# lucidrains/progen

Measured on NVIDIA H100. Metric: tokens_per_sec, higher is better.
Workload: dtype bf16

## Files before the change

### progen_b200/csrc/attn_wgmma.cu

```cuda
#include <cuda.h>
#include "common.cuh"
#include "tc_ptx.cuh"
#include "../../include/progen_b200.h"

namespace {

using namespace tc;

constexpr int DH = 64;
constexpr int TILE = 64;
constexpr int TILE_BYTES = TILE * DH * 2;
constexpr float LOG2E = 1.4426950408889634f;
constexpr float LN2 = 0.6931471805599453f;
constexpr int SMEM_BYTES = 1024  + 2 * TILE_BYTES + 2 * 2 * TILE_BYTES + 64;

struct Dims {
  int n, w, h;
  const float* rot_sin;
  const float* rot_cos;
};

__device__ __forceinline__ float quad_max(float v) {
  v = fmaxf(v, __shfl_xor_sync(0xffffffffu, v, 1));
  return fmaxf(v, __shfl_xor_sync(0xffffffffu, v, 2));
}
__device__ __forceinline__ float quad_sum(float v) {
  v += __shfl_xor_sync(0xffffffffu, v, 1);
  return v + __shfl_xor_sync(0xffffffffu, v, 2);
}
__device__ __forceinline__ uint32_t unrotate_pack(const Dims& dm, int pos, int jj, float d0, float d1) {
  if (dm.rot_sin) {
    const float s = __ldg(dm.rot_sin + pos * (DH / 2) + jj), c = __ldg(dm.rot_cos + pos * (DH / 2) + jj);
    const float a = d0 * c + d1 * s, b = d1 * c - d0 * s;
    d0 = a; d1 = b;
  }
  return pack_bf16x2(d0, d1);
}
template <int R> __device__ __forceinline__ void zero(float (&a)[R]) {
#pragma unroll
  for (int i = 0; i < R; ++i) a[i] = 0.f;
}
__device__ __forceinline__ void acc_to_a(uint32_t (&a)[4][4], const float (&s)[32]) {
#pragma unroll
  for (int kk = 0; kk < 4; ++kk)
#pragma unroll
    for (int i = 0; i < 4; ++i) a[kk][i] = pack_bf16x2(s[8 * kk + 2 * i], s[8 * kk + 2 * i + 1]);
}
__device__ __forceinline__ void issue_a_xt(float (&acc)[32], uint32_t a, uint32_t x) {
#pragma unroll
  for (int kk = 0; kk < 4; ++kk) wgmma_m64n64k16_ss<0>(acc, make_smem_desc<false>(a + 32 * kk), make_smem_desc<false>(x + 32 * kk));
}
__device__ __forceinline__ void issue_p_x(float (&acc)[32], const uint32_t (&p)[4][4], uint32_t x) {
#pragma unroll
  for (int kk = 0; kk < 4; ++kk) wgmma_m64n64k16_rs<1>(acc, p[kk], make_smem_desc<true>(x + 2048 * kk));
}
template <int R> __device__ __forceinline__ void mma_begin(float (&acc)[R]) {
  fence_regs(acc);
  wgmma_fence();
}
template <int R> __device__ __forceinline__ void mma_end(float (&acc)[R]) {
  wgmma_commit();
  wgmma_wait<0>();
  fence_regs(acc);
}

struct Smem {
  uint32_t fixed0, fixed1, ring, bars;
  __device__ Smem(uint8_t* raw) {
    fixed0 = (smem_u32(raw) + 1023u) & ~1023u;
    fixed1 = fixed0 + TILE_BYTES;
    ring = fixed1 + TILE_BYTES;
    bars = ring + 4 * TILE_BYTES;
  }
  __device__ uint32_t a(int st) const { return ring + st * 2 * TILE_BYTES; }
  __device__ uint32_t b(int st) const { return a(st) + TILE_BYTES; }
  __device__ uint32_t fixed_bar() const { return bars; }
  __device__ uint32_t full(int st) const { return bars + 8 + 8 * st; }
};

__device__ __forceinline__ void init_bars(const Smem& sm) {
  if (threadIdx.x == 0) {
    mbar_init(sm.fixed_bar(), 1);
    mbar_init(sm.full(0), 1);
    mbar_init(sm.full(1), 1);
    fence_barrier_init();
  }
  __syncthreads();
}

__global__ void __launch_bounds__(128) attn_fwd_wgmma_kernel(const __grid_constant__ CUtensorMap tm_qkv, bf16* __restrict__ out,
                                                             float* __restrict__ lse, const Dims dm) {
  extern __shared__ uint8_t smem_raw[];
  const Smem sm(smem_raw);
  const int tid = threadIdx.x, lane = tid & 31, warp = tid >> 5;
  const int g = lane >> 2, t4 = lane & 3;
  const int b = blockIdx.z, hh = blockIdx.y;
  const int q0 = blockIdx.x * TILE, win = q0 / dm.w, i0 = q0 % dm.w;
  const int I = dm.h * DH;
  const int row0 = b * dm.n;
  const int nprev = win > 0 ? dm.w / TILE : 0;
  const int ntiles = nprev + (i0 + TILE) / TILE;
  auto key_pos = [&](int kt) { return kt < nprev ? (win - 1) * dm.w + kt * TILE : win * dm.w + (kt - nprev) * TILE; };
  auto issue = [&](int kt, int st) {
    mbar_expect_tx(sm.full(st), 2 * TILE_BYTES);
    tma_load_2d(sm.a(st), &tm_qkv, sm.full(st), I + hh * DH, row0 + key_pos(kt));
    tma_load_2d(sm.b(st), &tm_qkv, sm.full(st), 2 * I + hh * DH, row0 + key_pos(kt));
  };
  init_bars(sm);
  if (tid == 0) {
    prefetch_tensormap(&tm_qkv);
    mbar_expect_tx(sm.fixed_bar(), TILE_BYTES);
    tma_load_2d(sm.fixed0, &tm_qkv, sm.fixed_bar(), hh * DH, row0 + q0);
    for (int kt = 0; kt < 2 && kt < ntiles; ++kt) issue(kt, kt);
  }

  const float sc = 0.125f  * LOG2E;
  float m_run[2], l_run[2];
  m_run[0] = m_run[1] = (win == 0) ? 0.f : -INFINITY;
  l_run[0] = l_run[1] = (win == 0) ? (float)dm.w : 0.f;
  float o[32];
  zero(o);
  const int qi_lo = i0 + warp * 16;
  mbar_wait(sm.fixed_bar(), 0);

  for (int kt = 0; kt < ntiles; ++kt) {
    const int st = kt & 1;
    mbar_wait(sm.full(st), (kt >> 1) & 1);
    float s[32];
    zero(s);
    mma_begin(s);
    issue_a_xt(s, sm.fixed0, sm.a(st));
    mma_end(s);
    const int c0 = (kt - nprev) * TILE;
    const bool need_mask = kt >= nprev && c0 + TILE - 1 > qi_lo;
    float tmax[2] = {-INFINITY, -INFINITY};
#pragma unroll
    for (int i = 0; i < 32; ++i) {
      float v = s[i] * sc;
      if (need_mask) {
        const int kj = c0 + 8 * (i >> 2) + 2 * t4 + (i & 1);
        const int qi = qi_lo + g + (((i >> 1) & 1) << 3);
        if (kj > qi) v = -INFINITY;
      }
      s[i] = v;
      tmax[(i >> 1) & 1] = fmaxf(tmax[(i >> 1) & 1], v);
    }
    float corr[2], rsum[2] = {0.f, 0.f};
#pragma unroll
    for (int r = 0; r < 2; ++r) {
      const float mn = fmaxf(m_run[r], quad_max(tmax[r]));
      corr[r] = exp2f(m_run[r] - mn);
      m_run[r] = mn;
    }
#pragma unroll
    for (int i = 0; i < 32; ++i) {
      const float p = exp2f(s[i] - m_run[(i >> 1) & 1]);
      s[i] = p;
      rsum[(i >> 1) & 1] += p;
    }
#pragma unroll
    for (int r = 0; r < 2; ++r) l_run[r] = l_run[r] * corr[r] + quad_sum(rsum[r]);
#pragma unroll
    for (int i = 0; i < 32; ++i) o[i] *= corr[(i >> 1) & 1];
    uint32_t pa[4][4];
    acc_to_a(pa, s);
    mma_begin(o);
    issue_p_x(o, pa, sm.b(st));
    mma_end(o);
    __syncthreads();
    if (tid == 0 && kt + 2 < ntiles) {
      fence_proxy_async();
      issue(kt + 2, st);
    }
  }
#pragma unroll
  for (int r = 0; r < 2; ++r) {
    const long long t = (long long)row0 + q0 + warp * 16 + g + 8 * r;
    const float inv = 1.f / l_run[r];
    bf16* op = out + t * I + hh * DH + 2 * t4;
#pragma unroll
    for (int j = 0; j < 8; ++j)
      *reinterpret_cast<uint32_t*>(op + 8 * j) = pack_bf16x2(o[4 * j + 2 * r] * inv, o[4 * j + 2 * r + 1] * inv);
    if (t4 == 0) lse[t * dm.h + hh] = m_run[r] * LN2 + logf(l_run[r]);
  }
}

__global__ void __launch_bounds__(128) attn_bwd_dq_wgmma_kernel(const __grid_constant__ CUtensorMap tm_qkv,
                                                                const __grid_constant__ CUtensorMap tm_do,
                                                                const bf16* __restrict__ out, const bf16* __restrict__ dout,
                                                                const float* __restrict__ lse, float* __restrict__ delta,
                                                                bf16* __restrict__ dqkv, const Dims dm) {
  extern __shared__ uint8_t smem_raw[];
  const Smem sm(smem_raw);
  const int tid = threadIdx.x, lane = tid & 31, warp = tid >> 5;
  const int g = lane >> 2, t4 = lane & 3;
  const int b = blockIdx.z, hh = blockIdx.y;
  const int q0 = blockIdx.x * TILE, win = q0 / dm.w, i0 = q0 % dm.w;
  const int I = dm.h * DH;
  const long long ld = 3LL * I;
  const int row0 = b * dm.n;
  const int nprev = win > 0 ? dm.w / TILE : 0;
  const int ntiles = nprev + (i0 + TILE) / TILE;
  auto key_pos = [&](int kt) { return kt < nprev ? (win - 1) * dm.w + kt * TILE : win * dm.w + (kt - nprev) * TILE; };
  auto issue = [&](int kt, int st) {
    mbar_expect_tx(sm.full(st), 2 * TILE_BYTES);
    tma_load_2d(sm.a(st), &tm_qkv, sm.full(st), I + hh * DH, row0 + key_pos(kt));
    tma_load_2d(sm.b(st), &tm_qkv, sm.full(st), 2 * I + hh * DH, row0 + key_pos(kt));
  };
  init_bars(sm);
  if (tid == 0) {
    prefetch_tensormap(&tm_qkv);
    prefetch_tensormap(&tm_do);
    mbar_expect_tx(sm.fixed_bar(), 2 * TILE_BYTES);
    tma_load_2d(sm.fixed0, &tm_qkv, sm.fixed_bar(), hh * DH, row0 + q0);
    tma_load_2d(sm.fixed1, &tm_do, sm.fixed_bar(), hh * DH, row0 + q0);
    for (int kt = 0; kt < 2 && kt < ntiles; ++kt) issue(kt, kt);
  }

  const float scale = 0.125f ;
  const float sc = scale * LOG2E;
  float L2[2], Dl[2];
#pragma unroll
  for (int r = 0; r < 2; ++r) {
    const long long t = (long long)row0 + q0 + warp * 16 + g + 8 * r;
    L2[r] = lse[t * dm.h + hh] * LOG2E;
    float acc = 0.f;
#pragma unroll
    for (int j = 0; j < 8; ++j) {
      const uint32_t ov = *reinterpret_cast<const uint32_t*>(out + t * I + hh * DH + 8 * j + 2 * t4);
      const uint32_t dv = *reinterpret_cast<const uint32_t*>(dout + t * I + hh * DH + 8 * j + 2 * t4);
      const float2 fo = __bfloat1622float2(*reinterpret_cast<const __nv_bfloat162*>(&ov));
      const float2 fd = __bfloat1622float2(*reinterpret_cast<const __nv_bfloat162*>(&dv));
      acc += fo.x * fd.x + fo.y * fd.y;
    }
    Dl[r] = quad_sum(acc);
    if (t4 == 0) delta[t * dm.h + hh] = Dl[r];
  }
  float dq[32];
  zero(dq);
  const int qi_lo = i0 + warp * 16;
  mbar_wait(sm.fixed_bar(), 0);

  for (int kt = 0; kt < ntiles; ++kt) {
    const int st = kt & 1;
    mbar_wait(sm.full(st), (kt >> 1) & 1);
    float s[32], dp[32];
    zero(s);
    zero(dp);
    fence_regs(dp);
    mma_begin(s);
    issue_a_xt(s, sm.fixed0, sm.a(st));
    issue_a_xt(dp, sm.fixed1, sm.b(st));
    mma_end(s);
    fence_regs(dp);
    const int c0 = (kt - nprev) * TILE;
    const bool need_mask = kt >= nprev && c0 + TILE - 1 > qi_lo;
#pragma unroll
    for (int i = 0; i < 32; ++i) {
      const int r = (i >> 1) & 1;
      float p = exp2f(s[i] * sc - L2[r]);
      if (need_mask) {
        const int kj = c0 + 8 * (i >> 2) + 2 * t4 + (i & 1);
        const int qi = qi_lo + g + (r << 3);
        if (kj > qi) p = 0.f;
      }
      s[i] = p * (dp[i] - Dl[r]) * scale;
    }
    uint32_t dsa[4][4];
    acc_to_a(dsa, s);
    mma_begin(dq);
    issue_p_x(dq, dsa, sm.a(st));
    mma_end(dq);
    __syncthreads();
    if (tid == 0 && kt + 2 < ntiles) {
      fence_proxy_async();
      issue(kt + 2, st);
    }
  }
#pragma unroll
  for (int r = 0; r < 2; ++r) {
    const int pos = q0 + warp * 16 + g + 8 * r;
    bf16* op = dqkv + ((long long)row0 + pos) * ld + hh * DH + 2 * t4;
#pragma unroll
    for (int j = 0; j < 8; ++j)
      *reinterpret_cast<uint32_t*>(op + 8 * j) = unrotate_pack(dm, pos, 4 * j + t4, dq[4 * j + 2 * r], dq[4 * j + 2 * r + 1]);
  }
}

__global__ void __launch_bounds__(128) attn_bwd_dkv_wgmma_kernel(const __grid_constant__ CUtensorMap tm_qkv,
                                                                 const __grid_constant__ CUtensorMap tm_do,
                                                                 const float* __restrict__ lse, const float* __restrict__ delta,
                                                                 bf16* __restrict__ dqkv, const Dims dm) {
  extern __shared__ uint8_t smem_raw[];
  const Smem sm(smem_raw);
  const int tid = threadIdx.x, lane = tid & 31, warp = tid >> 5;
  const int g = lane >> 2, t4 = lane & 3;
  const int b = blockIdx.z, hh = blockIdx.y;
  const int k0 = blockIdx.x * TILE, win = k0 / dm.w, j0 = k0 % dm.w;
  const int I = dm.h * DH;
  const long long ld = 3LL * I;
  const int row0 = b * dm.n;
  const int nwin = (dm.n + dm.w - 1) / dm.w;
  const int own_end = min((win + 1) * dm.w, dm.n);
  const int nown = (own_end - k0) / TILE;
  const int nnext = (win + 1 < nwin) ? (min((win + 2) * dm.w, dm.n) - own_end) / TILE : 0;
  const int ntiles = nown + nnext;
  auto q_pos = [&](int qt) { return qt < nown ? win * dm.w + j0 + qt * TILE : (win + 1) * dm.w + (qt - nown) * TILE; };
  auto issue = [&](int qt, int st) {
    mbar_expect_tx(sm.full(st), 2 * TILE_BYTES);
    tma_load_2d(sm.a(st), &tm_qkv, sm.full(st), hh * DH, row0 + q_pos(qt));
    tma_load_2d(sm.b(st), &tm_do, sm.full(st), hh * DH, row0 + q_pos(qt));
  };
  init_bars(sm);
  if (tid == 0) {
    prefetch_tensormap(&tm_qkv);
    prefetch_tensormap(&tm_do);
    mbar_expect_tx(sm.fixed_bar(), 2 * TILE_BYTES);
    tma_load_2d(sm.fixed0, &tm_qkv, sm.fixed_bar(), I + hh * DH, row0 + k0);
    tma_load_2d(sm.fixed1, &tm_qkv, sm.fixed_bar(), 2 * I + hh * DH, row0 + k0);
    for (int qt = 0; qt < 2 && qt < ntiles; ++qt) issue(qt, qt);
  }

  const float scale = 0.125f ;
  const float sc = scale * LOG2E;
  float dk[32], dv[32];
  zero(dk);
  zero(dv);
  const int kj_lo = j0 + warp * 16;
  mbar_wait(sm.fixed_bar(), 0);

  for (int qt = 0; qt < ntiles; ++qt) {
    const int st = qt & 1;
    const int qp = q_pos(qt);
    float Lq[16], Dq[16];
#pragma unroll
    for (int j = 0; j < 8; ++j)
#pragma unroll
      for (int c = 0; c < 2; ++c) {
        const long long t = (long long)row0 + qp + 8 * j + 2 * t4 + c;
        Lq[2 * j + c] = __ldg(lse + t * dm.h + hh) * LOG2E;
        Dq[2 * j + c] = __ldg(delta + t * dm.h + hh);
      }
    mbar_wait(sm.full(st), (qt >> 1) & 1);
    float s[32], dp[32];
    zero(s);
    zero(dp);
    fence_regs(dp);
    mma_begin(s);
    issue_a_xt(s, sm.fixed0, sm.a(st));
    issue_a_xt(dp, sm.fixed1, sm.b(st));
    mma_end(s);
    fence_regs(dp);
    const bool own = qt < nown;
    const int c0 = j0 + qt * TILE;
    const bool need_mask = own && c0 < kj_lo + 15;
#pragma unroll
    for (int i = 0; i < 32; ++i) {
      const int col = 8 * (i >> 2) + 2 * t4 + (i & 1);
      const int ci = 2 * (i >> 2) + (i & 1);
      float p = exp2f(s[i] * sc - Lq[ci]);
      if (need_mask) {
        const int qi = c0 + col;
        const int kj = kj_lo + g + (((i >> 1) & 1) << 3);
        if (kj > qi) p = 0.f;
      }
      dp[i] = p * (dp[i] - Dq[ci]) * scale;
      s[i] = p;
    }
    uint32_t pa[4][4], dsa[4][4];
    acc_to_a(pa, s);
    acc_to_a(dsa, dp);
    fence_regs(dk);
    mma_begin(dv);
    issue_p_x(dv, pa, sm.b(st));
    issue_p_x(dk, dsa, sm.a(st));
    mma_end(dv);
    fence_regs(dk);
    __syncthreads();
    if (tid == 0 && qt + 2 < ntiles) {
      fence_proxy_async();
      issue(qt + 2, st);
    }
  }
#pragma unroll
  for (int r = 0; r < 2; ++r) {
    const int pos = k0 + warp * 16 + g + 8 * r;
    bf16* pk = dqkv + ((long long)row0 + pos) * ld + I + hh * DH + 2 * t4;
    bf16* pv = pk + I;
#pragma unroll
    for (int j = 0; j < 8; ++j) {
      *reinterpret_cast<uint32_t*>(pk + 8 * j) = unrotate_pack(dm, pos, 4 * j + t4, dk[4 * j + 2 * r], dk[4 * j + 2 * r + 1]);
      *reinterpret_cast<uint32_t*>(pv + 8 * j) = unrotate_pack(dm, pos, 4 * j + t4, dv[4 * j + 2 * r], dv[4 * j + 2 * r + 1]);
    }
  }
}

template <typename K> int prepare(K kern) {
  static bool done = false;
  if (!done) {
    PG_CUDA(cudaFuncSetAttribute(kern, cudaFuncAttributeMaxDynamicSharedMemorySize, SMEM_BYTES));
    done = true;
  }
  return PROGEN_OK;
}

int check_dims(const void* qkv, int B, int seq_len, int window, int heads, int dim_head, bool full_windows) {
  PG_CHECK_ARG(qkv != nullptr && B > 0 && heads > 0 && dim_head == DH && window % TILE == 0 && seq_len > 0 &&
               seq_len % (full_windows ? window : TILE) == 0);
  PG_CHECK_ARG((long long)B * seq_len < (1ll << 31));
  return PROGEN_OK;
}

int bwd_tc(const void* qkv, const void* out, const void* dout, const float* lse, void* dqkv, float* delta,
           const float* rot_sin, const float* rot_cos, int B, int seq_len, int window, int heads, cudaStream_t s) {
  int rc;
  const int I = heads * DH;
  const uint64_t T = (uint64_t)B * seq_len;
  CUtensorMap tq, tdo;
  if ((rc = pg_tensor_map_2d_bf16(qkv, 3ull * I, T, 3ull * I, DH, TILE, &tq))) return rc;
  if ((rc = pg_tensor_map_2d_bf16(dout, (uint64_t)I, T, (uint64_t)I, DH, TILE, &tdo))) return rc;
  if ((rc = prepare(attn_bwd_dq_wgmma_kernel))) return rc;
  if ((rc = prepare(attn_bwd_dkv_wgmma_kernel))) return rc;
  const Dims dm{seq_len, window, heads, rot_sin, rot_cos};
  const dim3 grid(seq_len / TILE, heads, B);
  attn_bwd_dq_wgmma_kernel<<<grid, 128, SMEM_BYTES, s>>>(tq, tdo, (const bf16*)out, (const bf16*)dout, lse, delta, (bf16*)dqkv, dm);
  PG_LAUNCH_CHECK();
  attn_bwd_dkv_wgmma_kernel<<<grid, 128, SMEM_BYTES, s>>>(tq, tdo, lse, delta, (bf16*)dqkv, dm);
  PG_LAUNCH_CHECK();
  return PROGEN_OK;
}

}

extern "C" {

int progen_local_attn_fwd_tc(const void* qkv, void* out, float* lse, int B, int seq_len, int window, int heads, int dim_head,
                             void* stream) {
  int rc = check_dims(qkv, B, seq_len, window, heads, dim_head, false);
  if (rc) return rc;
  const int I = heads * DH;
  const uint64_t T = (uint64_t)B * seq_len;
  CUtensorMap tm;
  if ((rc = pg_tensor_map_2d_bf16(qkv, 3ull * I, T, 3ull * I, DH, TILE, &tm))) return rc;
  if ((rc = prepare(attn_fwd_wgmma_kernel))) return rc;
  const Dims dm{seq_len, window, heads, nullptr, nullptr};
  attn_fwd_wgmma_kernel<<<dim3(seq_len / TILE, heads, B), 128, SMEM_BYTES, (cudaStream_t)stream>>>(tm, (bf16*)out, lse, dm);
  PG_LAUNCH_CHECK();
  return PROGEN_OK;
}

int progen_local_attn_bwd_tc(const void* qkv, const void* out, const void* dout, const float* lse, void* dqkv, float* delta,
                             const float* rot_sin, const float* rot_cos, int B, int seq_len, int window, int heads, int dim_head,
                             void* stream) {
  const int rc = check_dims(qkv, B, seq_len, window, heads, dim_head, true);
  return rc ? rc : bwd_tc(qkv, out, dout, lse, dqkv, delta, rot_sin, rot_cos, B, seq_len, window, heads, (cudaStream_t)stream);
}

int progen_local_attn_bwd_cut_tc(const void* qkv, const void* out, const void* dout, const float* lse, void* dqkv,
                                 float* delta, const float* rot_sin, const float* rot_cos, int B, int seq_len, int window,
                                 int heads, int dim_head, void* stream) {
  const int rc = check_dims(qkv, B, seq_len, window, heads, dim_head, false);
  return rc ? rc : bwd_tc(qkv, out, dout, lse, dqkv, delta, rot_sin, rot_cos, B, seq_len, window, heads, (cudaStream_t)stream);
}

}
```

### progen_b200/csrc/gemm_tc.cu

```cuda
#include <cuda.h>
#include <algorithm>
#include <mutex>
#include <unordered_map>
#include "gemm.h"
#include "tc_ptx.cuh"

namespace {

using namespace tc;

constexpr int BM = 128;
constexpr int BN = 128;
constexpr int BK = 64;
constexpr int WG_K = 16;
constexpr int THREADS = 384;
constexpr int A_BYTES = BM * BK * 2;
constexpr int B_BYTES = BN * BK * 2;
constexpr int STAGE_BYTES = A_BYTES + B_BYTES;
constexpr int STAGES = 4;
constexpr int EPI_ROWS = 64;
constexpr int EPI_ITEMS = EPI_ROWS * (BN / 8) / 128;
constexpr int CS_LD = BN + 4;
constexpr int CS_BYTES = EPI_ROWS * CS_LD * 4;
constexpr int SMEM_TOTAL = 1024  + STAGES * STAGE_BYTES + 2 * CS_BYTES + 2 * STAGES * 8;
// ... 265 lines not shown

EncodeTiledFn get_encode_fn() {
  static EncodeTiledFn fn = nullptr;
  static std::once_flag once;
  std::call_once(once, [] {
    void* p = nullptr;
    cudaDriverEntryPointQueryResult q;
    if (cudaGetDriverEntryPoint("cuTensorMapEncodeTiled", &p, cudaEnableDefault, &q) == cudaSuccess &&
        q == cudaDriverEntryPointSuccess)
      fn = reinterpret_cast<EncodeTiledFn>(p);
  });
  return fn;
}

struct MapKey {
  const void* ptr; uint64_t inner, outer, stride; uint32_t box_inner, box_outer, elem_bytes, swizzle;
  bool operator==(const MapKey& o) const {
    return ptr == o.ptr && inner == o.inner && outer == o.outer && stride == o.stride && box_inner == o.box_inner &&
           box_outer == o.box_outer && elem_bytes == o.elem_bytes && swizzle == o.swizzle;
  }
};
struct MapKeyHash {
  size_t operator()(const MapKey& k) const {
    size_t h = std::hash<const void*>()(k.ptr);
    auto mix = [&](uint64_t v) { h ^= std::hash<uint64_t>()(v) + 0x9e3779b97f4a7c15ULL + (h << 6) + (h >> 2); };
    mix(k.inner); mix(k.outer); mix(k.stride); mix(k.box_inner); mix(k.box_outer); mix(k.elem_bytes * 256 + k.swizzle);
    return h;
  }
};

int get_tensor_map(const void* ptr, uint64_t inner, uint64_t outer, uint64_t row_stride_elems, uint32_t box_inner,
                   uint32_t box_outer, CUtensorMap* out, uint32_t elem_bytes = 2, uint32_t swizzle = 128) {
  static std::unordered_map<MapKey, CUtensorMap, MapKeyHash> cache;
  static std::mutex mu;
  MapKey key{ptr, inner, outer, row_stride_elems, box_inner, box_outer, elem_bytes, swizzle};
  std::lock_guard<std::mutex> lock(mu);
  auto it = cache.find(key);
  if (it != cache.end()) { *out = it->second; return PROGEN_OK; }
  EncodeTiledFn fn = get_encode_fn();
  if (!fn) { progen_set_error("cuTensorMapEncodeTiled driver entry point not found"); return PROGEN_ERR_DEVICE; }
  cuuint64_t dims[2] = {inner, outer};
  cuuint64_t strides[1] = {row_stride_elems * elem_bytes};
  const CUtensorMapSwizzle sw = swizzle == 128 ? CU_TENSOR_MAP_SWIZZLE_128B : swizzle == 64 ? CU_TENSOR_MAP_SWIZZLE_64B
                              : swizzle == 32 ? CU_TENSOR_MAP_SWIZZLE_32B : CU_TENSOR_MAP_SWIZZLE_NONE;
  cuuint32_t box[2] = {box_inner, box_outer};
  cuuint32_t estr[2] = {1, 1};
  CUtensorMap m;
  CUresult r = fn(&m, elem_bytes == 4 ? CU_TENSOR_MAP_DATA_TYPE_FLOAT32 : CU_TENSOR_MAP_DATA_TYPE_BFLOAT16, 2,
                  const_cast<void*>(ptr), dims, strides, box, estr, CU_TENSOR_MAP_INTERLEAVE_NONE, sw, CU_TENSOR_MAP_L2_PROMOTION_L2_256B,
                  CU_TENSOR_MAP_FLOAT_OOB_FILL_NONE);
  if (r != CUDA_SUCCESS) {
    progen_set_error("cuTensorMapEncodeTiled failed (CUresult %d) ptr=%p inner=%llu outer=%llu stride=%llu box=%ux%u", (int)r,
                     ptr, (unsigned long long)inner, (unsigned long long)outer, (unsigned long long)row_stride_elems,
                     box_inner, box_outer);
    return PROGEN_ERR_CUDA;
  }
  if (cache.size() > 4096) cache.clear();
  cache.emplace(key, m);
  *out = m;
  return PROGEN_OK;
}


template <bool A_MN, bool B_MN, int KIND, typename TO, bool TAIL>
int launch_inst(const CUtensorMap& ta, const CUtensorMap& tb, const CUtensorMap& ta2, const CUtensorMap& tb2,
                const GemmDev& gd, int tiles, cudaStream_t stream) {
  auto kern = gemm_tc_kernel<A_MN, B_MN, KIND, TO, TAIL>;
  static bool attr_set = false;
  if (!attr_set) {
    PG_CUDA(cudaFuncSetAttribute(kern, cudaFuncAttributeMaxDynamicSharedMemorySize, SMEM_TOTAL));
    attr_set = true;
  }
  kern<<<std::min(tiles, pg_num_sms()), THREADS, SMEM_TOTAL, stream>>>(ta, tb, ta2, tb2, gd, tiles);
  PG_LAUNCH_CHECK();
  return PROGEN_OK;
}

}

int pg_tensor_map_2d_bf16(const void* ptr, uint64_t inner, uint64_t outer, uint64_t row_stride_elems, uint32_t box_inner,
                          uint32_t box_outer, CUtensorMap* out) {
  return get_tensor_map(ptr, inner, outer, row_stride_elems, box_inner, box_outer, out);
}

int gemm_tc_launch(const GemmArgs& a, cudaStream_t stream) {
  PG_CHECK_ARG(a.in_dtype == PG_BF16);
  PG_CHECK_ARG(a.M > 0 && a.N > 0 && a.K > 0 && a.batch >= 1 && a.split_k >= 1);
  PG_CHECK_ARG(a.N % 8 == 0);
  PG_CHECK_ARG(a.K % BK == 0);
  PG_CHECK_ARG(a.lda % 8 == 0 && a.ldb % 8 == 0);
  PG_CHECK_ARG((reinterpret_cast<uintptr_t>(a.A) & 15) == 0 && (reinterpret_cast<uintptr_t>(a.B) & 15) == 0);
  PG_CHECK_ARG(!(a.split_k > 1 && a.causal));
  if (a.epi_kind == EPI_ROTARY) PG_CHECK_ARG(a.epi.seq_len % 32 == 0);
  PG_CHECK_ARG((reinterpret_cast<uintptr_t>(a.epi.colsum) & 15) == 0);
  PG_CHECK_ARG(!(a.split_k > 1 || a.batch_reduce) || (a.epi_kind == EPI_ACCUM && a.epi.atomic));
  PG_CHECK_TAIL(a);
  const bool tail = a.K2 > 0;
  if (tail) {
    PG_CHECK_ARG(a.K2 % 8 == 0 && a.lda2 % 8 == 0 && a.ldb2 % 8 == 0);
    PG_CHECK_ARG(a.a2_mn_major == a.a_mn_major && a.b2_mn_major == a.b_mn_major);
    PG_CHECK_ARG((reinterpret_cast<uintptr_t>(a.A2) & 15) == 0 && (reinterpret_cast<uintptr_t>(a.B2) & 15) == 0);
  }

  const uint64_t a_rows = (a.batch > 1 && a.a_batch_rows > 0) ? (uint64_t)a.a_batch_rows * a.batch
                                                              : (uint64_t)(a.a_mn_major ? a.K : a.M);
  const uint64_t b_rows = (a.batch > 1 && a.b_batch_rows > 0) ? (uint64_t)a.b_batch_rows * a.batch
                                                              : (uint64_t)(a.b_mn_major ? a.K : a.N);
  CUtensorMap ta, tb;
  int rc;
  if (!a.a_mn_major) rc = get_tensor_map(a.A, a.K, a_rows, a.lda, BK, BM, &ta);
  else               rc = get_tensor_map(a.A, a.M, a_rows, a.lda, 64, BK, &ta);
  if (rc) return rc;
  if (!a.b_mn_major) rc = get_tensor_map(a.B, a.K, b_rows, a.ldb, BK, BN, &tb);
  else               rc = get_tensor_map(a.B, a.N, b_rows, a.ldb, 64, BK, &tb);
  if (rc) return rc;
  CUtensorMap ta2 = ta, tb2 = tb;
  if (tail) {
    if (!a.a_mn_major) rc = get_tensor_map(a.A2, a.K2, a.M, a.lda2, BK, BM, &ta2);
    else               rc = get_tensor_map(a.A2, a.M, a.K2, a.lda2, 64, BK, &ta2);
    if (rc) return rc;
    if (!a.b_mn_major) rc = get_tensor_map(a.B2, a.K2, a.N, a.ldb2, BK, BN, &tb2);
    else               rc = get_tensor_map(a.B2, a.N, a.K2, a.ldb2, 64, BK, &tb2);
    if (rc) return rc;
  }

  GemmDev gd;
  gd.M = a.M; gd.N = a.N; gd.K = a.K;
  gd.batch = a.batch; gd.batch_reduce = a.batch_reduce;
  gd.a_batch_rows = (int)a.a_batch_rows; gd.b_batch_rows = (int)a.b_batch_rows; gd.d_batch_rows = a.d_batch_rows;
  gd.causal = a.causal; gd.split_k = a.split_k;
  gd.epi = a.epi;
  gd.K2 = a.K2;
  const long long tiles = (long long)a.batch * a.split_k * ((a.M + BM - 1) / BM) * ((a.N + BN - 1) / BN);
  PG_CHECK_ARG(tiles < (1ll << 31));

  const int am = a.a_mn_major ? 1 : 0, bm = a.b_mn_major ? 1 : 0;
  const bool obf = a.out_dtype == PG_BF16;
#define TC_CASE(AM, BMJ, KIND, TO)                                                                       \
  return tail ? launch_inst<AM, BMJ, KIND, TO, true>(ta, tb, ta2, tb2, gd, (int)tiles, stream)            \
              : launch_inst<AM, BMJ, KIND, TO, false>(ta, tb, ta2, tb2, gd, (int)tiles, stream)
  switch (a.epi_kind) {
    case EPI_STORE:
      if (!am && bm) { if (obf) TC_CASE(false, true, EPI_STORE, bf16); else TC_CASE(false, true, EPI_STORE, float); }
      if (!am && !bm) { if (obf) TC_CASE(false, false, EPI_STORE, bf16); else TC_CASE(false, false, EPI_STORE, float); }
      if (am && bm) { if (obf) TC_CASE(true, true, EPI_STORE, bf16); else TC_CASE(true, true, EPI_STORE, float); }
      break;
    case EPI_ROTARY:
      if (!am && bm && obf) TC_CASE(false, true, EPI_ROTARY, bf16);
      break;
    case EPI_RESIDUAL:
      if (!am && bm) TC_CASE(false, true, EPI_RESIDUAL, float);
      break;
    case EPI_GLU:
      if (!am && bm && obf) TC_CASE(false, true, EPI_GLU, bf16);
      break;
    case EPI_GELU:
      if (!am && bm && obf) TC_CASE(false, true, EPI_GELU, bf16);
      break;
    case EPI_GLU_BWD:
      if (!am && !bm && obf) TC_CASE(false, false, EPI_GLU_BWD, bf16);
      break;
    case EPI_GELU_BWD:
      if (!am && !bm && obf) TC_CASE(false, false, EPI_GELU_BWD, bf16);
      break;
    case EPI_ACCUM:
      if (am && bm) return launch_inst<true, true, EPI_ACCUM, float, false>(ta, tb, ta2, tb2, gd, (int)tiles, stream);
// ... 9 lines not shown
```

### progen_b200/csrc/tc_ptx.cuh

```cuda
#pragma once
#include <cuda.h>
#include "common.cuh"

namespace tc {

__device__ __forceinline__ uint32_t smem_u32(const void* p) { return (uint32_t)__cvta_generic_to_shared(p); }

__device__ __forceinline__ void mbar_init(uint32_t bar, uint32_t count) {
  asm volatile("mbarrier.init.shared::cta.b64 [%0], %1;" ::"r"(bar), "r"(count) : "memory");
}
__device__ __forceinline__ void mbar_expect_tx(uint32_t bar, uint32_t bytes) {
  asm volatile("mbarrier.arrive.expect_tx.shared::cta.b64 _, [%0], %1;" ::"r"(bar), "r"(bytes) : "memory");
}
__device__ __forceinline__ void mbar_arrive(uint32_t bar) {
  asm volatile("mbarrier.arrive.shared::cta.b64 _, [%0];" ::"r"(bar) : "memory");
}
__device__ __forceinline__ void mbar_wait(uint32_t bar, uint32_t parity) {
  uint32_t ok = 0, spins = 0;
  do {
    asm volatile(
        "{\n\t.reg .pred p;\n\t"
        "mbarrier.try_wait.parity.shared::cta.b64 p, [%1], %2;\n\t"
        "selp.u32 %0, 1, 0, p;\n\t}"
        : "=r"(ok) : "r"(bar), "r"(parity) : "memory");
    if (!ok && ++spins > (1u << 26)) __trap();
  } while (!ok);
}
__device__ __forceinline__ void fence_barrier_init() { asm volatile("fence.mbarrier_init.release.cluster;" ::: "memory"); }
__device__ __forceinline__ void fence_proxy_async() { asm volatile("fence.proxy.async.shared::cta;" ::: "memory"); }

__device__ __forceinline__ void tma_load_2d(uint32_t dst, const CUtensorMap* map, uint32_t bar, int c0, int c1) {
  asm volatile(
      "cp.async.bulk.tensor.2d.shared::cluster.global.mbarrier::complete_tx::bytes [%0], [%1, {%3, %4}], [%2];"
      ::"r"(dst), "l"(map), "r"(bar), "r"(c0), "r"(c1) : "memory");
}
__device__ __forceinline__ void prefetch_tensormap(const CUtensorMap* map) {
  asm volatile("prefetch.tensormap [%0];" ::"l"(map) : "memory");
}

template <bool MN_MAJOR>
__device__ __forceinline__ uint64_t make_smem_desc(uint32_t smem_addr, uint32_t lbo_bytes = 8192) {
  uint64_t d = 0;
  d |= (uint64_t)((smem_addr & 0x3FFFF) >> 4);
  d |= (uint64_t)(MN_MAJOR ? (lbo_bytes >> 4) : 1) << 16;
  d |= (uint64_t)(1024 >> 4) << 32;
  d |= (uint64_t)1 << 62;
  return d;
}

__device__ __forceinline__ void wgmma_fence() { asm volatile("wgmma.fence.sync.aligned;" ::: "memory"); }
__device__ __forceinline__ void wgmma_commit() { asm volatile("wgmma.commit_group.sync.aligned;" ::: "memory"); }
template <int N> __device__ __forceinline__ void wgmma_wait() { asm volatile("wgmma.wait_group.sync.aligned %0;" ::"n"(N) : "memory"); }
template <int R> __device__ __forceinline__ void fence_regs(float (&d)[R]) {
#pragma unroll
  for (int i = 0; i < R; ++i) asm volatile("" : "+f"(d[i])::"memory");
}

template <int TA, int TB>
__device__ __forceinline__ void wgmma_m64n128k16_bf16(float (&d)[64], uint64_t adesc, uint64_t bdesc) {
  asm volatile(
      "{\n\t"
      "wgmma.mma_async.sync.aligned.m64n128k16.f32.bf16.bf16 "
      "{%0, %1, %2, %3, %4, %5, %6, %7, %8, %9, %10, %11, %12, %13, %14, %15, %16, %17, %18, %19, %20, %21, %22, %23, "
      "%24, %25, %26, %27, %28, %29, %30, %31, %32, %33, %34, %35, %36, %37, %38, %39, %40, %41, %42, %43, %44, %45, %46, "
      "%47, %48, %49, %50, %51, %52, %53, %54, %55, %56, %57, %58, %59, %60, %61, %62, %63}, "
      "%64, %65, 1, 1, 1, %66, %67;\n\t}"
      : "+f"(d[0]), "+f"(d[1]), "+f"(d[2]), "+f"(d[3]), "+f"(d[4]), "+f"(d[5]), "+f"(d[6]), "+f"(d[7]), "+f"(d[8]),
        "+f"(d[9]), "+f"(d[10]), "+f"(d[11]), "+f"(d[12]), "+f"(d[13]), "+f"(d[14]), "+f"(d[15]), "+f"(d[16]),
        "+f"(d[17]), "+f"(d[18]), "+f"(d[19]), "+f"(d[20]), "+f"(d[21]), "+f"(d[22]), "+f"(d[23]), "+f"(d[24]),
        "+f"(d[25]), "+f"(d[26]), "+f"(d[27]), "+f"(d[28]), "+f"(d[29]), "+f"(d[30]), "+f"(d[31]), "+f"(d[32]),
        "+f"(d[33]), "+f"(d[34]), "+f"(d[35]), "+f"(d[36]), "+f"(d[37]), "+f"(d[38]), "+f"(d[39]), "+f"(d[40]),
        "+f"(d[41]), "+f"(d[42]), "+f"(d[43]), "+f"(d[44]), "+f"(d[45]), "+f"(d[46]), "+f"(d[47]), "+f"(d[48]),
        "+f"(d[49]), "+f"(d[50]), "+f"(d[51]), "+f"(d[52]), "+f"(d[53]), "+f"(d[54]), "+f"(d[55]), "+f"(d[56]),
        "+f"(d[57]), "+f"(d[58]), "+f"(d[59]), "+f"(d[60]), "+f"(d[61]), "+f"(d[62]), "+f"(d[63])
      : "l"(adesc), "l"(bdesc), "n"(TA), "n"(TB));
}

template <int TB>
__device__ __forceinline__ void wgmma_m64n64k16_ss(float (&d)[32], uint64_t adesc, uint64_t bdesc) {
  asm volatile(
      "{\n\t"
      "wgmma.mma_async.sync.aligned.m64n64k16.f32.bf16.bf16 "
      "{%0, %1, %2, %3, %4, %5, %6, %7, %8, %9, %10, %11, %12, %13, %14, %15, %16, %17, %18, %19, %20, %21, %22, %23, %24, %25, %26, %27, %28, %29, %30, %31}, "
      "%32, %33, 1, 1, 1, 0, %34;\n\t}"
      : "+f"(d[0]), "+f"(d[1]), "+f"(d[2]), "+f"(d[3]), "+f"(d[4]), "+f"(d[5]), "+f"(d[6]), "+f"(d[7]), "+f"(d[8]), "+f"(d[9]), "+f"(d[10]), "+f"(d[11]), "+f"(d[12]), "+f"(d[13]), "+f"(d[14]), "+f"(d[15]), "+f"(d[16]), "+f"(d[17]), "+f"(d[18]), "+f"(d[19]), "+f"(d[20]), "+f"(d[21]), "+f"(d[22]), "+f"(d[23]), "+f"(d[24]), "+f"(d[25]), "+f"(d[26]), "+f"(d[27]), "+f"(d[28]), "+f"(d[29]), "+f"(d[30]), "+f"(d[31])
      : "l"(adesc), "l"(bdesc), "n"(TB));
}
template <int TB>
__device__ __forceinline__ void wgmma_m64n64k16_rs(float (&d)[32], const uint32_t (&a)[4], uint64_t bdesc) {
  asm volatile(
      "{\n\t"
      "wgmma.mma_async.sync.aligned.m64n64k16.f32.bf16.bf16 "
      "{%0, %1, %2, %3, %4, %5, %6, %7, %8, %9, %10, %11, %12, %13, %14, %15, %16, %17, %18, %19, %20, %21, %22, %23, %24, %25, %26, %27, %28, %29, %30, %31}, "
      "{%32, %33, %34, %35}, %36, 1, 1, 1, %37;\n\t}"
      : "+f"(d[0]), "+f"(d[1]), "+f"(d[2]), "+f"(d[3]), "+f"(d[4]), "+f"(d[5]), "+f"(d[6]), "+f"(d[7]), "+f"(d[8]), "+f"(d[9]), "+f"(d[10]), "+f"(d[11]), "+f"(d[12]), "+f"(d[13]), "+f"(d[14]), "+f"(d[15]), "+f"(d[16]), "+f"(d[17]), "+f"(d[18]), "+f"(d[19]), "+f"(d[20]), "+f"(d[21]), "+f"(d[22]), "+f"(d[23]), "+f"(d[24]), "+f"(d[25]), "+f"(d[26]), "+f"(d[27]), "+f"(d[28]), "+f"(d[29]), "+f"(d[30]), "+f"(d[31])
      : "r"(a[0]), "r"(a[1]), "r"(a[2]), "r"(a[3]), "l"(bdesc), "n"(TB));
}

}

int pg_tensor_map_2d_bf16(const void* ptr, uint64_t inner, uint64_t outer, uint64_t row_stride_elems, uint32_t box_inner,
                          uint32_t box_outer, CUtensorMap* out);
```

Before: 1.008 million.

## Replace block syncs with empty mbarriers and TMA-load lse/delta in attention backward

Replaces the per-tile __syncthreads plus refill in the attention kernels with per-stage empty mbarriers, so TMA refills for freed stages are issued while wgmma work is still in flight. The forward PV wgmma is left uncommitted-waited across iterations, and the first QK^T wgmma uses scale-d=0 to skip zeroing accumulators. The dK/dV kernel gets three stages and, when heads divide by 4, loads lse/delta tiles by TMA into shared memory instead of strided __ldg gathers. This adds barrier complexity, more shared memory per block (possibly lowering occupancy), and a second kernel variant.

```diff
diff --git a/progen_b200/csrc/attn_wgmma.cu b/progen_b200/csrc/attn_wgmma.cu
--- a/progen_b200/csrc/attn_wgmma.cu
+++ b/progen_b200/csrc/attn_wgmma.cu
@@ -12,7 +12,8 @@
 constexpr int TILE_BYTES = TILE * DH * 2;
 constexpr float LOG2E = 1.4426950408889634f;
 constexpr float LN2 = 0.6931471805599453f;
-constexpr int SMEM_BYTES = 1024  + 2 * TILE_BYTES + 2 * 2 * TILE_BYTES + 64;
+constexpr int LD_HEADS = 4;
+constexpr int LD_BYTES = TILE * LD_HEADS * 4;
 
 struct Dims {
   int n, w, h;
@@ -46,9 +47,10 @@
 #pragma unroll
     for (int i = 0; i < 4; ++i) a[kk][i] = pack_bf16x2(s[8 * kk + 2 * i], s[8 * kk + 2 * i + 1]);
 }
-__device__ __forceinline__ void issue_a_xt(float (&acc)[32], uint32_t a, uint32_t x) {
-#pragma unroll
-  for (int kk = 0; kk < 4; ++kk) wgmma_m64n64k16_ss<0>(acc, make_smem_desc<false>(a + 32 * kk), make_smem_desc<false>(x + 32 * kk));
+template <bool ACC = true> __device__ __forceinline__ void issue_a_xt(float (&acc)[32], uint32_t a, uint32_t x) {
+  wgmma_m64n64k16_ss<0, ACC>(acc, make_smem_desc<false>(a), make_smem_desc<false>(x));
+#pragma unroll
+  for (int kk = 1; kk < 4; ++kk) wgmma_m64n64k16_ss<0>(acc, make_smem_desc<false>(a + 32 * kk), make_smem_desc<false>(x + 32 * kk));
 }
 __device__ __forceinline__ void issue_p_x(float (&acc)[32], const uint32_t (&p)[4][4], uint32_t x) {
 #pragma unroll
@@ -64,34 +66,65 @@
   fence_regs(acc);
 }
 
+template <int FIXED, int STAGES, bool LD = false>
 struct Smem {
+  static constexpr int STAGE_BYTES = 2 * TILE_BYTES + (LD ? 2 * LD_BYTES : 0);
+  static constexpr int BYTES = 1024  + FIXED * TILE_BYTES + STAGES * STAGE_BYTES + 8 * (1 + 2 * STAGES);
   uint32_t fixed0, fixed1, ring, bars;
   __device__ Smem(uint8_t* raw) {
     fixed0 = (smem_u32(raw) + 1023u) & ~1023u;
     fixed1 = fixed0 + TILE_BYTES;
-    ring = fixed1 + TILE_BYTES;
-    bars = ring + 4 * TILE_BYTES;
+    ring = fixed0 + FIXED * TILE_BYTES;
+    bars = ring + STAGES * STAGE_BYTES;
   }
   __device__ uint32_t a(int st) const { return ring + st * 2 * TILE_BYTES; }
   __device__ uint32_t b(int st) const { return a(st) + TILE_BYTES; }
+  __device__ uint32_t lse(int st) const { return ring + STAGES * 2 * TILE_BYTES + st * 2 * LD_BYTES; }
+  __device__ uint32_t delta(int st) const { return lse(st) + LD_BYTES; }
   __device__ uint32_t fixed_bar() const { return bars; }
   __device__ uint32_t full(int st) const { return bars + 8 + 8 * st; }
+  __device__ uint32_t empty(int st) const { return bars + 8 + 8 * (STAGES + st); }
+
+  __device__ void init_bars() const {
+    if (threadIdx.x == 0) {
+      mbar_init(fixed_bar(), 1);
+      for (int st = 0; st < STAGES; ++st) {
+        mbar_init(full(st), 1);
+        mbar_init(empty(st), 128);
+      }
+      fence_barrier_init();
+    }
+    __syncthreads();
+  }
+  template <typename F> __device__ void release_previous(int t, int ntiles, F&& issue) const {
+    const int j = t - 1;
+    if (j < 0) return;
+    mbar_arrive(empty(j % STAGES));
+    if (threadIdx.x == 0 && j + STAGES < ntiles) {
+      mbar_wait(empty(j % STAGES), (j / STAGES) & 1);
+      fence_proxy_async();
+      issue(j + STAGES, j % STAGES);
+    }
+    __syncwarp();
+  }
+  template <typename F> __device__ void refill(int t, int ntiles, F&& issue) const {
+    const int j = t - 1;
+    if (j >= 0 && j + STAGES < ntiles) {
+      mbar_wait(empty(j % STAGES), (j / STAGES) & 1);
+      fence_proxy_async();
+      issue(j + STAGES, j % STAGES);
+    }
+  }
+  __device__ void release(int t) const { mbar_arrive(empty(t % STAGES)); }
+  __device__ void wait_full(int t) const { mbar_wait(full(t % STAGES), (t / STAGES) & 1); }
 };
 
-__device__ __forceinline__ void init_bars(const Smem& sm) {
-  if (threadIdx.x == 0) {
-    mbar_init(sm.fixed_bar(), 1);
-    mbar_init(sm.full(0), 1);
-    mbar_init(sm.full(1), 1);
-    fence_barrier_init();
-  }
-  __syncthreads();
-}
+constexpr int FWD_STAGES = 2, DQ_STAGES = 2, DKV_STAGES = 3;
 
 __global__ void __launch_bounds__(128) attn_fwd_wgmma_kernel(const __grid_constant__ CUtensorMap tm_qkv, bf16* __restrict__ out,
                                                              float* __restrict__ lse, const Dims dm) {
   extern __shared__ uint8_t smem_raw[];
-  const Smem sm(smem_raw);
+  const Smem<1, FWD_STAGES> sm(smem_raw);
   const int tid = threadIdx.x, lane = tid & 31, warp = tid >> 5;
   const int g = lane >> 2, t4 = lane & 3;
   const int b = blockIdx.z, hh = blockIdx.y;
@@ -106,12 +139,12 @@
     tma_load_2d(sm.a(st), &tm_qkv, sm.full(st), I + hh * DH, row0 + key_pos(kt));
     tma_load_2d(sm.b(st), &tm_qkv, sm.full(st), 2 * I + hh * DH, row0 + key_pos(kt));
   };
-  init_bars(sm);
+  sm.init_bars();
   if (tid == 0) {
     prefetch_tensormap(&tm_qkv);
     mbar_expect_tx(sm.fixed_bar(), TILE_BYTES);
     tma_load_2d(sm.fixed0, &tm_qkv, sm.fixed_bar(), hh * DH, row0 + q0);
-    for (int kt = 0; kt < 2 && kt < ntiles; ++kt) issue(kt, kt);
+    for (int kt = 0; kt < FWD_STAGES && kt < ntiles; ++kt) issue(kt, kt);
   }
 
   const float sc = 0.125f  * LOG2E;
@@ -124,13 +157,16 @@
   mbar_wait(sm.fixed_bar(), 0);
 
   for (int kt = 0; kt < ntiles; ++kt) {
-    const int st = kt & 1;
-    mbar_wait(sm.full(st), (kt >> 1) & 1);
+    const int st = kt % FWD_STAGES;
+    sm.wait_full(kt);
     float s[32];
-    zero(s);
     mma_begin(s);
-    issue_a_xt(s, sm.fixed0, sm.a(st));
-    mma_end(s);
+    issue_a_xt<false>(s, sm.fixed0, sm.a(st));
+    wgmma_commit();
+    wgmma_wait<0>();
+    fence_regs(s);
+    fence_regs(o);
+    sm.release_previous(kt, ntiles, issue);
     const int c0 = (kt - nprev) * TILE;
     const bool need_mask = kt >= nprev && c0 + TILE - 1 > qi_lo;
     float tmax[2] = {-INFINITY, -INFINITY};
@@ -166,13 +202,10 @@
     acc_to_a(pa, s);
     mma_begin(o);
     issue_p_x(o, pa, sm.b(st));
-    mma_end(o);
-    __syncthreads();
-    if (tid == 0 && kt + 2 < ntiles) {
-      fence_proxy_async();
-      issue(kt + 2, st);
-    }
-  }
+    wgmma_commit();
+  }
+  wgmma_wait<0>();
+  fence_regs(o);
 #pragma unroll
   for (int r = 0; r < 2; ++r) {
     const long long t = (long long)row0 + q0 + warp * 16 + g + 8 * r;
@@ -191,7 +224,7 @@
                                                                 const float* __restrict__ lse, float* __restrict__ delta,
                                                                 bf16* __restrict__ dqkv, const Dims dm) {
   extern __shared__ uint8_t smem_raw[];
-  const Smem sm(smem_raw);
+  const Smem<2, DQ_STAGES> sm(smem_raw);
   const int tid = threadIdx.x, lane = tid & 31, warp = tid >> 5;
   const int g = lane >> 2, t4 = lane & 3;
   const int b = blockIdx.z, hh = blockIdx.y;
@@ -207,14 +240,14 @@
     tma_load_2d(sm.a(st), &tm_qkv, sm.full(st), I + hh * DH, row0 + key_pos(kt));
     tma_load_2d(sm.b(st), &tm_qkv, sm.full(st), 2 * I + hh * DH, row0 + key_pos(kt));
   };
-  init_bars(sm);
+  sm.init_bars();
   if (tid == 0) {
     prefetch_tensormap(&tm_qkv);
     prefetch_tensormap(&tm_do);
     mbar_expect_tx(sm.fixed_bar(), 2 * TILE_BYTES);
     tma_load_2d(sm.fixed0, &tm_qkv, sm.fixed_bar(), hh * DH, row0 + q0);
     tma_load_2d(sm.fixed1, &tm_do, sm.fixed_bar(), hh * DH, row0 + q0);
-    for (int kt = 0; kt < 2 && kt < ntiles; ++kt) issue(kt, kt);
+    for (int kt = 0; kt < DQ_STAGES && kt < ntiles; ++kt) issue(kt, kt);
   }
 
   const float scale = 0.125f ;
@@ -242,8 +275,8 @@
   mbar_wait(sm.fixed_bar(), 0);
 
   for (int kt = 0; kt < ntiles; ++kt) {
-    const int st = kt & 1;
-    mbar_wait(sm.full(st), (kt >> 1) & 1);
+    const int st = kt % DQ_STAGES;
+    sm.wait_full(kt);
     float s[32], dp[32];
     zero(s);
     zero(dp);
@@ -251,7 +284,11 @@
     mma_begin(s);
     issue_a_xt(s, sm.fixed0, sm.a(st));
     issue_a_xt(dp, sm.fixed1, sm.b(st));
-    mma_end(s);
+    wgmma_commit();
+    if (tid == 0) sm.refill(kt, ntiles, issue);
+    __syncwarp();
+    wgmma_wait<0>();
+    fence_regs(s);
     fence_regs(dp);
     const int c0 = (kt - nprev) * TILE;
     const bool need_mask = kt >= nprev && c0 + TILE - 1 > qi_lo;
@@ -271,11 +308,7 @@
     mma_begin(dq);
     issue_p_x(dq, dsa, sm.a(st));
     mma_end(dq);
-    __syncthreads();
-    if (tid == 0 && kt + 2 < ntiles) {
-      fence_proxy_async();
-      issue(kt + 2, st);
-    }
+    sm.release(kt);
   }
 #pragma unroll
   for (int r = 0; r < 2; ++r) {
@@ -287,12 +320,15 @@
   }
 }
 
+template <bool LD>
 __global__ void __launch_bounds__(128) attn_bwd_dkv_wgmma_kernel(const __grid_constant__ CUtensorMap tm_qkv,
                                                                  const __grid_constant__ CUtensorMap tm_do,
+                                                                 const __grid_constant__ CUtensorMap tm_lse,
+                                                                 const __grid_constant__ CUtensorMap tm_delta,
                                                                  const float* __restrict__ lse, const float* __restrict__ delta,
                                                                  bf16* __restrict__ dqkv, const Dims dm) {
   extern __shared__ uint8_t smem_raw[];
-  const Smem sm(smem_raw);
+  const Smem<2, DKV_STAGES, LD> sm(smem_raw);
   const int tid = threadIdx.x, lane = tid & 31, warp = tid >> 5;
   const int g = lane >> 2, t4 = lane & 3;
   const int b = blockIdx.z, hh = blockIdx.y;
@@ -307,19 +343,28 @@
   const int ntiles = nown + nnext;
   auto q_pos = [&](int qt) { return qt < nown ? win * dm.w + j0 + qt * TILE : (win + 1) * dm.w + (qt - nown) * TILE; };
   auto issue = [&](int qt, int st) {
-    mbar_expect_tx(sm.full(st), 2 * TILE_BYTES);
+    mbar_expect_tx(sm.full(st), 2 * TILE_BYTES + (LD ? 2 * LD_BYTES : 0));
     tma_load_2d(sm.a(st), &tm_qkv, sm.full(st), hh * DH, row0 + q_pos(qt));
     tma_load_2d(sm.b(st), &tm_do, sm.full(st), hh * DH, row0 + q_pos(qt));
+    if (LD) {
+      tma_load_2d(sm.lse(st), &tm_lse, sm.full(st), hh & ~(LD_HEADS - 1), row0 + q_pos(qt));
+      tma_load_2d(sm.delta(st), &tm_delta, sm.full(st), hh & ~(LD_HEADS - 1), row0 + q_pos(qt));
+    }
   };
-  init_bars(sm);
+  sm.init_bars();
   if (tid == 0) {
     prefetch_tensormap(&tm_qkv);
     prefetch_tensormap(&tm_do);
+    if (LD) {
+      prefetch_tensormap(&tm_lse);
+      prefetch_tensormap(&tm_delta);
+    }
     mbar_expect_tx(sm.fixed_bar(), 2 * TILE_BYTES);
     tma_load_2d(sm.fixed0, &tm_qkv, sm.fixed_bar(), I + hh * DH, row0 + k0);
     tma_load_2d(sm.fixed1, &tm_qkv, sm.fixed_bar(), 2 * I + hh * DH, row0 + k0);
-    for (int qt = 0; qt < 2 && qt < ntiles; ++qt) issue(qt, qt);
-  }
+    for (int qt = 0; qt < DKV_STAGES && qt < ntiles; ++qt) issue(qt, qt);
+  }
+  const float* ld_lse = reinterpret_cast<const float*>(smem_raw + (sm.lse(0) - smem_u32(smem_raw))) + (hh & (LD_HEADS - 1));
 
   const float scale = 0.125f ;
   const float sc = scale * LOG2E;
@@ -330,18 +375,20 @@
   mbar_wait(sm.fixed_bar(), 0);
 
   for (int qt = 0; qt < ntiles; ++qt) {
-    const int st = qt & 1;
-    const int qp = q_pos(qt);
-    float Lq[16], Dq[16];
-#pragma unroll
-    for (int j = 0; j < 8; ++j)
-#pragma unroll
-      for (int c = 0; c < 2; ++c) {
-        const long long t = (long long)row0 + qp + 8 * j + 2 * t4 + c;
-        Lq[2 * j + c] = __ldg(lse + t * dm.h + hh) * LOG2E;
-        Dq[2 * j + c] = __ldg(delta + t * dm.h + hh);
-      }
-    mbar_wait(sm.full(st), (qt >> 1) & 1);
+    const int st = qt % DKV_STAGES;
+    float Lq[LD ? 1 : 16], Dq[LD ? 1 : 16];
+    if (!LD) {
+      const int qp = q_pos(qt);
+#pragma unroll
+      for (int j = 0; j < 8; ++j)
+#pragma unroll
+        for (int c = 0; c < 2; ++c) {
+          const long long t = (long long)row0 + qp + 8 * j + 2 * t4 + c;
+          Lq[2 * j + c] = __ldg(lse + t * dm.h + hh) * LOG2E;
+          Dq[2 * j + c] = __ldg(delta + t * dm.h + hh);
+        }
+    }
+    sm.wait_full(qt);
     float s[32], dp[32];
     zero(s);
     zero(dp);
@@ -349,8 +396,14 @@
     mma_begin(s);
     issue_a_xt(s, sm.fixed0, sm.a(st));
     issue_a_xt(dp, sm.fixed1, sm.b(st));
-    mma_end(s);
+    wgmma_commit();
+    if (tid == 0) sm.refill(qt, ntiles, issue);
+    __syncwarp();
+    wgmma_wait<0>();
+    fence_regs(s);
     fence_regs(dp);
+    const float* st_lse = ld_lse + st * (2 * LD_BYTES / 4);
+    const float* st_delta = st_lse + LD_BYTES / 4;
     const bool own = qt < nown;
     const int c0 = j0 + qt * TILE;
     const bool need_mask = own && c0 < kj_lo + 15;
@@ -358,13 +411,15 @@
     for (int i = 0; i < 32; ++i) {
       const int col = 8 * (i >> 2) + 2 * t4 + (i & 1);
       const int ci = 2 * (i >> 2) + (i & 1);
-      float p = exp2f(s[i] * sc - Lq[ci]);
+      const float lq = LD ? st_lse[col * LD_HEADS] * LOG2E : Lq[LD ? 0 : ci];
+      const float dq = LD ? st_delta[col * LD_HEADS] : Dq[LD ? 0 : ci];
+      float p = exp2f(s[i] * sc - lq);
       if (need_mask) {
         const int qi = c0 + col;
         const int kj = kj_lo + g + (((i >> 1) & 1) << 3);
         if (kj > qi) p = 0.f;
       }
-      dp[i] = p * (dp[i] - Dq[ci]) * scale;
+      dp[i] = p * (dp[i] - dq) * scale;
       s[i] = p;
     }
     uint32_t pa[4][4], dsa[4][4];
@@ -376,11 +431,7 @@
     issue_p_x(dk, dsa, sm.a(st));
     mma_end(dv);
     fence_regs(dk);
-    __syncthreads();
-    if (tid == 0 && qt + 2 < ntiles) {
-      fence_proxy_async();
-      issue(qt + 2, st);
-    }
+    sm.release(qt);
   }
 #pragma unroll
   for (int r = 0; r < 2; ++r) {
@@ -395,14 +446,16 @@
   }
 }
 
-template <typename K> int prepare(K kern) {
+template <auto KERN> int prepare(int smem_bytes) {
   static bool done = false;
   if (!done) {
-    PG_CUDA(cudaFuncSetAttribute(kern, cudaFuncAttributeMaxDynamicSharedMemorySize, SMEM_BYTES));
+    PG_CUDA(cudaFuncSetAttribute(KERN, cudaFuncAttributeMaxDynamicSharedMemorySize, smem_bytes));
     done = true;
   }
   return PROGEN_OK;
 }
+constexpr int FWD_SMEM = Smem<1, FWD_STAGES>::BYTES, DQ_SMEM = Smem<2, DQ_STAGES>::BYTES;
+template <bool LD> constexpr int DKV_SMEM = Smem<2, DKV_STAGES, LD>::BYTES;
 
 int check_dims(const void* qkv, int B, int seq_len, int window, int heads, int dim_head, bool full_windows) {
   PG_CHECK_ARG(qkv != nullptr && B > 0 && heads > 0 && dim_head == DH && window % TILE == 0 && seq_len > 0 &&
@@ -419,13 +472,23 @@
   CUtensorMap tq, tdo;
   if ((rc = pg_tensor_map_2d_bf16(qkv, 3ull * I, T, 3ull * I, DH, TILE, &tq))) return rc;
   if ((rc = pg_tensor_map_2d_bf16(dout, (uint64_t)I, T, (uint64_t)I, DH, TILE, &tdo))) return rc;
-  if ((rc = prepare(attn_bwd_dq_wgmma_kernel))) return rc;
-  if ((rc = prepare(attn_bwd_dkv_wgmma_kernel))) return rc;
+  const bool ld = heads % LD_HEADS == 0 && ((uintptr_t)lse & 15) == 0 && ((uintptr_t)delta & 15) == 0;
+  CUtensorMap tl = tq, td = tq;
+  if (ld) {
+    if ((rc = pg_tensor_map_2d_f32(lse, (uint64_t)heads, T, (uint64_t)heads, LD_HEADS, TILE, &tl))) return rc;
+    if ((rc = pg_tensor_map_2d_f32(delta, (uint64_t)heads, T, (uint64_t)heads, LD_HEADS, TILE, &td))) return rc;
+  }
+  if ((rc = prepare<attn_bwd_dq_wgmma_kernel>(DQ_SMEM))) return rc;
+  if ((rc = prepare<attn_bwd_dkv_wgmma_kernel<true>>(DKV_SMEM<true>))) return rc;
+  if ((rc = prepare<attn_bwd_dkv_wgmma_kernel<false>>(DKV_SMEM<false>))) return rc;
   const Dims dm{seq_len, window, heads, rot_sin, rot_cos};
   const dim3 grid(seq_len / TILE, heads, B);
-  attn_bwd_dq_wgmma_kernel<<<grid, 128, SMEM_BYTES, s>>>(tq, tdo, (const bf16*)out, (const bf16*)dout, lse, delta, (bf16*)dqkv, dm);
+  attn_bwd_dq_wgmma_kernel<<<grid, 128, DQ_SMEM, s>>>(tq, tdo, (const bf16*)out, (const bf16*)dout, lse, delta, (bf16*)dqkv, dm);
   PG_LAUNCH_CHECK();
-  attn_bwd_dkv_wgmma_kernel<<<grid, 128, SMEM_BYTES, s>>>(tq, tdo, lse, delta, (bf16*)dqkv, dm);
+  if (ld)
+    attn_bwd_dkv_wgmma_kernel<true><<<grid, 128, DKV_SMEM<true>, s>>>(tq, tdo, tl, td, lse, delta, (bf16*)dqkv, dm);
+  else
+    attn_bwd_dkv_wgmma_kernel<false><<<grid, 128, DKV_SMEM<false>, s>>>(tq, tdo, tl, td, lse, delta, (bf16*)dqkv, dm);
   PG_LAUNCH_CHECK();
   return PROGEN_OK;
 }
@@ -442,9 +505,9 @@
   const uint64_t T = (uint64_t)B * seq_len;
   CUtensorMap tm;
   if ((rc = pg_tensor_map_2d_bf16(qkv, 3ull * I, T, 3ull * I, DH, TILE, &tm))) return rc;
-  if ((rc = prepare(attn_fwd_wgmma_kernel))) return rc;
+  if ((rc = prepare<attn_fwd_wgmma_kernel>(FWD_SMEM))) return rc;
   const Dims dm{seq_len, window, heads, nullptr, nullptr};
-  attn_fwd_wgmma_kernel<<<dim3(seq_len / TILE, heads, B), 128, SMEM_BYTES, (cudaStream_t)stream>>>(tm, (bf16*)out, lse, dm);
+  attn_fwd_wgmma_kernel<<<dim3(seq_len / TILE, heads, B), 128, FWD_SMEM, (cudaStream_t)stream>>>(tm, (bf16*)out, lse, dm);
   PG_LAUNCH_CHECK();
   return PROGEN_OK;
 }
diff --git a/progen_b200/csrc/gemm_tc.cu b/progen_b200/csrc/gemm_tc.cu
--- a/progen_b200/csrc/gemm_tc.cu
+++ b/progen_b200/csrc/gemm_tc.cu
@@ -371,6 +371,10 @@
                           uint32_t box_outer, CUtensorMap* out) {
   return get_tensor_map(ptr, inner, outer, row_stride_elems, box_inner, box_outer, out);
 }
+int pg_tensor_map_2d_f32(const void* ptr, uint64_t inner, uint64_t outer, uint64_t row_stride_elems, uint32_t box_inner,
+                         uint32_t box_outer, CUtensorMap* out) {
+  return get_tensor_map(ptr, inner, outer, row_stride_elems, box_inner, box_outer, out, 4, 0);
+}
 
 int gemm_tc_launch(const GemmArgs& a, cudaStream_t stream) {
   PG_CHECK_ARG(a.in_dtype == PG_BF16);
diff --git a/progen_b200/csrc/tc_ptx.cuh b/progen_b200/csrc/tc_ptx.cuh
--- a/progen_b200/csrc/tc_ptx.cuh
+++ b/progen_b200/csrc/tc_ptx.cuh
@@ -76,15 +76,23 @@
       : "l"(adesc), "l"(bdesc), "n"(TA), "n"(TB));
 }
 
-template <int TB>
+template <int TB, int ACC = 1>
 __device__ __forceinline__ void wgmma_m64n64k16_ss(float (&d)[32], uint64_t adesc, uint64_t bdesc) {
-  asm volatile(
-      "{\n\t"
-      "wgmma.mma_async.sync.aligned.m64n64k16.f32.bf16.bf16 "
-      "{%0, %1, %2, %3, %4, %5, %6, %7, %8, %9, %10, %11, %12, %13, %14, %15, %16, %17, %18, %19, %20, %21, %22, %23, %24, %25, %26, %27, %28, %29, %30, %31}, "
-      "%32, %33, 1, 1, 1, 0, %34;\n\t}"
-      : "+f"(d[0]), "+f"(d[1]), "+f"(d[2]), "+f"(d[3]), "+f"(d[4]), "+f"(d[5]), "+f"(d[6]), "+f"(d[7]), "+f"(d[8]), "+f"(d[9]), "+f"(d[10]), "+f"(d[11]), "+f"(d[12]), "+f"(d[13]), "+f"(d[14]), "+f"(d[15]), "+f"(d[16]), "+f"(d[17]), "+f"(d[18]), "+f"(d[19]), "+f"(d[20]), "+f"(d[21]), "+f"(d[22]), "+f"(d[23]), "+f"(d[24]), "+f"(d[25]), "+f"(d[26]), "+f"(d[27]), "+f"(d[28]), "+f"(d[29]), "+f"(d[30]), "+f"(d[31])
-      : "l"(adesc), "l"(bdesc), "n"(TB));
+#define PG_WGMMA_SS_N64(OUT, SCALE_D)                                                                                     \
+  asm volatile(                                                                                                         \
+      "{\n\t"                                                                                                            \
+      "wgmma.mma_async.sync.aligned.m64n64k16.f32.bf16.bf16 "                                                            \
+      "{%0, %1, %2, %3, %4, %5, %6, %7, %8, %9, %10, %11, %12, %13, %14, %15, %16, %17, %18, %19, %20, %21, %22, %23, "  \
+      "%24, %25, %26, %27, %28, %29, %30, %31}, "                                                                        \
+      "%32, %33, " SCALE_D ", 1, 1, 0, %34;\n\t}"                                                                        \
+      : OUT(d[0]), OUT(d[1]), OUT(d[2]), OUT(d[3]), OUT(d[4]), OUT(d[5]), OUT(d[6]), OUT(d[7]), OUT(d[8]), OUT(d[9]),   \
+        OUT(d[10]), OUT(d[11]), OUT(d[12]), OUT(d[13]), OUT(d[14]), OUT(d[15]), OUT(d[16]), OUT(d[17]), OUT(d[18]),      \
+        OUT(d[19]), OUT(d[20]), OUT(d[21]), OUT(d[22]), OUT(d[23]), OUT(d[24]), OUT(d[25]), OUT(d[26]), OUT(d[27]),      \
+        OUT(d[28]), OUT(d[29]), OUT(d[30]), OUT(d[31])                                                                   \
+      : "l"(adesc), "l"(bdesc), "n"(TB))
+  if constexpr (ACC) PG_WGMMA_SS_N64("+f", "1");
+  else PG_WGMMA_SS_N64("=f", "0");
+#undef PG_WGMMA_SS_N64
 }
 template <int TB>
 __device__ __forceinline__ void wgmma_m64n64k16_rs(float (&d)[32], const uint32_t (&a)[4], uint64_t bdesc) {
@@ -101,3 +109,5 @@
 
 int pg_tensor_map_2d_bf16(const void* ptr, uint64_t inner, uint64_t outer, uint64_t row_stride_elems, uint32_t box_inner,
                           uint32_t box_outer, CUtensorMap* out);
+int pg_tensor_map_2d_f32(const void* ptr, uint64_t inner, uint64_t outer, uint64_t row_stride_elems, uint32_t box_inner,
+                         uint32_t box_outer, CUtensorMap* out);
```

Measured after the change: 1.019 million, median of 6. +1.1%, better.
